# montib/rays1bench

Hardware: AMD Instinct MI355X
Metric: mrays/s on 'large' scene 1200x800x10spp (higher is better)
Workload: dtype f32

## Files before the change

include/rays1.h:

```cpp
#ifndef RAYS1_H
#define RAYS1_H

#include <stddef.h>
#include <stdint.h>

#ifdef __cplusplus
extern "C" {
#endif

#define R1_ABI_VERSION 4

enum
{
    R1_OK = 0,
    R1_EINVAL = -1,
    R1_ENODEVICE = -2,
    R1_EHIP = -3,
    R1_ENOMEM = -4,
    R1_ELIMIT = -5
};

enum
{
    R1_MAT_LAMBERTIAN = 0,
// ... 148 lines not shown


typedef struct r1_multi r1_multi;
int r1_multi_create(int32_t n_devices, const int32_t *devices, r1_multi **out);
void r1_multi_destroy(r1_multi *m);
int r1_multi_set_scene(r1_multi *m, const r1_scene *scene, const r1_camera *camera);
int r1_multi_set_camera(r1_multi *m, const r1_camera *camera);
int r1_multi_render(r1_multi *m, const r1_params *params, uint8_t *rgb_out, uint64_t *num_rays_out, double *device_seconds_out);
int r1_multi_render_async(r1_multi *m, const r1_params *params, void *host_frame);
int r1_multi_render_batch_async(r1_multi *m, const r1_params *params, int32_t n_frames, uint32_t seed_stride, void *host_frames);
int r1_multi_sync(r1_multi *m);
typedef struct r1_multi_layout_info
{
    size_t block_bytes;
    size_t record_bytes;
    size_t count_offset;
    size_t send_bytes;
    size_t gathered_bytes;
    size_t frame_record_bytes;
    size_t frame_count_offset;
    size_t host_bytes;
    size_t counts_pitch;
} r1_multi_layout_info;
int r1_multi_layout(const r1_params *params, int32_t n_devices, int32_t n_frames, r1_multi_layout_info *out);
int r1_multi_info(r1_multi *m, int32_t *n_devices, int32_t *rccl_version, r1_launch_info *first_device);


typedef struct r1_bvh_info
{
    int32_t nodes, leaves, depth, stack_entries, spheres, pairs;
    float centre[3];
    int32_t pad_local;
    int32_t root_leaf;
} r1_bvh_info;
int r1_bvh_describe(const r1_scene *scene, int32_t leaf_max, r1_bvh_info *info, float *nodes_out, size_t nodes_cap, uint32_t *ids_out,
                    size_t ids_cap);

typedef struct r1_grid_info
{
    float lo[3], hi[3];
    int32_t cells[3];
    float cell[3];
    float pad;
    float v_safe;
    float centre_lo[3], centre_hi[3];
    int32_t spheres;
    int32_t outliers;
    int32_t registrations;
    int32_t max_occupancy;
    float build_ms;
} r1_grid_info;
int r1_grid_describe(const r1_scene *scene, r1_grid_info *info, uint32_t *start_out, size_t start_cap, uint32_t *ids_out, size_t ids_cap,
                     uint32_t *outliers_out, size_t outliers_cap);

int r1_grid_visit(const r1_scene *scene, const float o[3], const float d[3], uint32_t *presented, size_t cap, size_t *n_presented,
                  int32_t *hit_index, float *hit_t, int32_t *fallback);

enum
{
    R1_SCENE_SMALL = 0,
    R1_SCENE_MEDIUM = 1,
    R1_SCENE_LARGE = 2,
    R1_SCENE_GRID = 3
};

typedef struct r1_host_scene r1_host_scene;
// ... 22 lines not shown
```

rays1bench_amd/binding.py:

```python
import ctypes as C
import os
import sys
import subprocess
import time

import numpy as np

_lib = None
HERE = os.path.dirname(os.path.abspath(__file__))
CSRC = os.path.join(HERE, "csrc")
LIBDIR = os.path.join(HERE, "lib")

R1_OK, R1_EINVAL, R1_ENODEVICE, R1_EHIP, R1_ENOMEM, R1_ELIMIT = 0, -1, -2, -3, -4, -5
SCENE_SMALL, SCENE_MEDIUM, SCENE_LARGE, SCENE_GRID = 0, 1, 2, 3
VARIANT_DEFAULT, VARIANT_REFERENCE, VARIANT_PREFILTER, VARIANT_STATS, VARIANT_BVH, VARIANT_BVH_STATS, VARIANT_WAVEFRONT = 0, 1, 2, 3, 4, 5, 6
VARIANT_GRID, VARIANT_GRID_STATS = 7, 8



def _stream_arg(stream_ptr):
    if stream_ptr:
        return C.c_void_p(stream_ptr)
    torch = sys.modules.get("torch")
    if torch is not None and torch.cuda.is_available() and torch.cuda.is_initialized():
# ... 13 lines not shown
    ] + [("mat_type", C.POINTER(C.c_uint8))] + [
        (n, C.POINTER(C.c_float)) for n in ("albedo_r", "albedo_g", "albedo_b", "mat_param")
    ]


class CCamera(C.Structure):
    _fields_ = [(n, C.c_float * 3) for n in ("origin", "lower_left", "horizontal", "vertical", "u", "v", "w")] + [
        ("lens_radius", C.c_float)
    ]


class Params(C.Structure):
    _fields_ = [
        ("width", C.c_int32), ("height", C.c_int32), ("spp", C.c_int32), ("max_bounces", C.c_int32),
        ("seed", C.c_uint32), ("tile_w", C.c_int32), ("tile_h", C.c_int32),
        ("shard", C.c_int32), ("num_shards", C.c_int32), ("variant", C.c_int32),
    ]


class MultiLayout(C.Structure):
    _fields_ = [(k, C.c_size_t) for k in ("block_bytes", "record_bytes", "count_offset", "send_bytes", "gathered_bytes", "frame_record_bytes",
                                          "frame_count_offset", "host_bytes", "counts_pitch")]


class LaunchInfo(C.Structure):
    _fields_ = [("compute_units", C.c_int32), ("blocks", C.c_int32), ("threads_per_block", C.c_int32),
                ("spheres_active", C.c_int32), ("spheres_padded", C.c_int32), ("groups", C.c_int32), ("samples", C.c_uint64),
                ("kernel", C.c_int32), ("bvh_nodes", C.c_int32), ("bvh_leaves", C.c_int32), ("bvh_depth", C.c_int32),
                ("tiles_in_kernel", C.c_int32)]


class BvhInfo(C.Structure):
    _fields_ = [("nodes", C.c_int32), ("leaves", C.c_int32), ("depth", C.c_int32), ("stack_entries", C.c_int32), ("spheres", C.c_int32),
                ("pairs", C.c_int32), ("centre", C.c_float * 3), ("pad_local", C.c_int32), ("root_leaf", C.c_int32)]


def make_params(width, height, spp, seed=10001, max_bounces=50, tile_w=32, tile_h=32, shard=0, num_shards=1, variant=0):
    return Params(width, height, spp, max_bounces, seed, tile_w, tile_h, shard, num_shards, variant)


_lib_path = os.path.join(LIBDIR, "librays1.so")


def lib_path():
    return _lib_path


def set_lib_path(path):
    global _lib_path
    if _lib is not None:
        raise R1Error(R1_EINVAL, "set_lib_path after the library was loaded")
    _lib_path = os.path.abspath(path)


def build(verbose=False):
    subprocess.check_call(["make", "-j4", "-C", CSRC] + ([] if verbose else ["-s"]))


class GridInfo(C.Structure):
    _fields_ = [("lo", C.c_float * 3), ("hi", C.c_float * 3), ("cells", C.c_int32 * 3), ("cell", C.c_float * 3), ("pad", C.c_float),
                ("v_safe", C.c_float), ("centre_lo", C.c_float * 3), ("centre_hi", C.c_float * 3), ("spheres", C.c_int32),
                ("outliers", C.c_int32), ("registrations", C.c_int32), ("max_occupancy", C.c_int32), ("build_ms", C.c_float)]


_u8p, _f32p, _u64p, _i32p, _dblp = (C.POINTER(t) for t in (C.c_uint8, C.c_float, C.c_uint64, C.c_int32, C.c_double))
_ctx = C.c_void_p
SYMBOLS = [
# ... 428 lines not shown


def shard_block_bytes(params):
    return int(lib().r1_shard_block_bytes(C.byref(params)))


def frame_record_bytes(params):
    return int(lib().r1_frame_record_bytes(C.byref(params)))


def shard_record_bytes(params):
    return int(lib().r1_shard_record_bytes(C.byref(params)))


def tile_count(params):
    a, b = C.c_int32(), C.c_int32()
    _check(lib().r1_tile_count(C.byref(params), C.byref(a), C.byref(b)))
    return int(a.value), int(b.value)


def multi_layout(params, n_devices, n_frames=1):
    out = MultiLayout()
    _check(lib().r1_multi_layout(C.byref(params), n_devices, n_frames, C.byref(out)))
    return {k: int(getattr(out, k)) for k, _ in MultiLayout._fields_}


def bvh_describe(cscene, leaf_max=0):
    info = BvhInfo()
    _check(lib().r1_bvh_describe(C.byref(cscene), leaf_max, C.byref(info), None, 0, None, 0))
    nodes = np.zeros((info.nodes, 16), np.float32)
    ids = np.zeros(max(2 * info.pairs, 2), np.uint32)
    _check(lib().r1_bvh_describe(C.byref(cscene), leaf_max, C.byref(info), nodes.ctypes.data_as(_f32p), nodes.size,
                                 ids.ctypes.data_as(C.POINTER(C.c_uint32)), ids.size))
    d = {k: int(getattr(info, k)) for k, _ in BvhInfo._fields_ if k != "centre"}
    d["centre"] = np.array(list(info.centre), np.float32)
    return d, nodes, ids[:2 * info.pairs]


def grid_describe(cscene):
    info = GridInfo()
    _check(lib().r1_grid_describe(C.byref(cscene), C.byref(info), None, 0, None, 0, None, 0))
    ncells = int(info.cells[0]) * int(info.cells[1]) * int(info.cells[2])
    start = np.zeros(ncells + 1, np.uint32)
    ids = np.zeros(max(info.registrations, 1), np.uint32)
    outl = np.zeros(max(info.outliers, 1), np.uint32)
    u32p = C.POINTER(C.c_uint32)
    _check(lib().r1_grid_describe(C.byref(cscene), C.byref(info), start.ctypes.data_as(u32p), start.size, ids.ctypes.data_as(u32p), ids.size,
                                  outl.ctypes.data_as(u32p), outl.size))
    d = {}
    for k, t in GridInfo._fields_:
        v = getattr(info, k)
        d[k] = np.array(list(v), np.float32 if k != "cells" else np.int64) if hasattr(v, "__len__") else v
    return d, start, ids[:info.registrations], outl[:info.outliers]


def grid_visit(cscene, o, d, cap=1 << 16):
    o = np.ascontiguousarray(o, np.float32)
    d = np.ascontiguousarray(d, np.float32)
    pres = np.zeros(cap, np.uint32)
    n, hi, ht, fb = C.c_size_t(), C.c_int32(), C.c_float(), C.c_int32()
    _check(lib().r1_grid_visit(C.byref(cscene), o.ctypes.data_as(_f32p), d.ctypes.data_as(_f32p), pres.ctypes.data_as(C.POINTER(C.c_uint32)), cap,
                               C.byref(n), C.byref(hi), C.byref(ht), C.byref(fb)))
    if n.value > cap:
        return grid_visit(cscene, o, d, int(n.value))
    return pres[:n.value], int(hi.value), float(ht.value), bool(fb.value)


# ... 47 lines not shown
```

rays1bench_amd/csrc/r1_bvh.cpp:

```cpp
#include <hip/hip_runtime.h>

#include "r1_device.h"
#include "../../include/rays1.h"

#include <algorithm>
#include <cmath>
#include <cstdint>
#include <cstdlib>
#include <cstring>
#include <vector>

struct R1Bvh
{
    std::vector<float> nodes;
    std::vector<float> prims;
    std::vector<uint32_t> ids;
    int max_depth = 0;
    uint32_t n_leaves = 0;
    float centre[3] = {0, 0, 0};
    int pad_local = 0;
    int root_leaf = 0;
};

namespace
{

struct Box
{
    double lo[3], hi[3];
    double clo[3], chi[3];
    double kmax;
    double rmax;
    double floor_pad;
    void clear()
    {
        for (int a = 0; a < 3; ++a)
            lo[a] = clo[a] = 1e300, hi[a] = chi[a] = -1e300;
        kmax = rmax = floor_pad = 0;
    }
    void merge(const Box &b)
    {
        for (int a = 0; a < 3; ++a)
        {
            lo[a] = std::min(lo[a], b.lo[a]), hi[a] = std::max(hi[a], b.hi[a]);
            clo[a] = std::min(clo[a], b.clo[a]), chi[a] = std::max(chi[a], b.chi[a]);
        }
        kmax = std::max(kmax, b.kmax), rmax = std::max(rmax, b.rmax), floor_pad = std::max(floor_pad, b.floor_pad);
    }
    double area() const
    {
        const double dx = hi[0] - lo[0], dy = hi[1] - lo[1], dz = hi[2] - lo[2];
        return dx * dy + dy * dz + dz * dx;
    }
};
// ... 164 lines not shown
            }
        }
        if (mid <= b || mid >= e)
        {
            mid = b + n / 2;
            const int a = axis;
            std::nth_element(order.begin() + b, order.begin() + mid, order.begin() + e, [&](uint32_t p, uint32_t q) {
                return sphere[p].clo[a] < sphere[q].clo[a] || (sphere[p].clo[a] == sphere[q].clo[a] && p < q);
            });
        }

        const uint32_t node = (uint32_t)(out->nodes.size() / 16);
        out->nodes.resize(out->nodes.size() + 16);
        out->max_depth = std::max(out->max_depth, depth + 1);
        const Box b0 = bound(b, mid), b1 = bound(mid, e);
        const uint32_t c0 = build(b, mid, depth + 1, b0);
        const uint32_t c1 = build(mid, e, depth + 1, b1);
        fill(node, b0, c0, b1, c1);
        return node;
    }

    void fill(uint32_t node, const Box &b0, uint32_t c0, const Box &b1, uint32_t c1)
    {
        float m0[3], e0[3], m1[3], e1[3];
        double w0, k0, w1, k1;
        encode(b0, m0, e0, w0, k0);
        encode(b1, m1, e1, w1, k1);
        float *p = &out->nodes[16 * (size_t)node];
        const double u = ldexp(1.0, -24), w2 = std::max(w0, w1), k = std::max(k0, k1);
        const double head = 1.0 + ldexp(1.0, -18);
        float A, K;
        if (!pad_local)
        {
            double g2 = 0;
            for (const float *m : {m0, m1})
            {
                double q = 0;
                for (int a = 0; a < 3; ++a)
                    q += ((double)m[a] - centre[a]) * ((double)m[a] - centre[a]);
                g2 = std::max(g2, q);
            }
            const double c1n = std::fabs(centre[0]) + std::fabs(centre[1]) + std::fabs(centre[2]);
            A = round_up((2.0 * w2 + u) * head), K = round_up((k + 2.0 * w2 * g2 + u * (1.0 + c1n)) * head);
        }
        else
        {
            double g2 = 0, mn2 = 0, M = 0, M0 = 0, M1 = 0;
            for (int a = 0; a < 3; ++a)
            {
                const double h = 0.5 * ((double)m0[a] - (double)m1[a]), mn = 0.5 * ((double)m0[a] + (double)m1[a]);
                g2 += h * h, mn2 += mn * mn;
                M0 = std::max(M0, std::fabs((double)m0[a])), M1 = std::max(M1, std::fabs((double)m1[a]));
            }
            M = M0 + M1;
            const double eps = std::min(1.0, std::max(1.0 / 64.0, std::sqrt(g2) / d_typ));
            const double a_loc = (0.25 * (1.0 + eps) * w2 + u / 8.0) * (1.0 + ldexp(1.0, -10));
            A = round_up(a_loc * head);
            K = round_up((k + (1.0 + 1.0 / eps) * w2 * g2 + u * (0.5 + std::sqrt(mn2)) + a_loc * 3075.0 * 288.0 * u * u * M * M) * head);
        }
        p[0] = m0[0], p[1] = m1[0], p[2] = m0[1], p[3] = m1[1];
        p[4] = m0[2], p[5] = m1[2], p[6] = e0[0], p[7] = e1[0];
        p[8] = e0[1], p[9] = e1[1], p[10] = e0[2], p[11] = e1[2];
        p[12] = A, p[13] = K;
        memcpy(&p[14], &c0, 4);
        memcpy(&p[15], &c1, 4);
    }
};

}

void r1_build_bvh(uint32_t na, const float *cx, const float *cy, const float *cz, const float *rsq, const double *rbound, int leaf_max,
                  R1Bvh &out)
{
    out.nodes.clear(), out.prims.clear(), out.ids.clear();
    out.max_depth = 0, out.n_leaves = 0;
    if (leaf_max < 1)
// ... 141 lines not shown
                }
            }
            if (order_new.size() == nn)
            {
                std::vector<uint32_t> new_of(nn);
                for (uint32_t i = 0; i < nn; ++i)
                    new_of[order_new[i]] = i;
                std::vector<float> moved(out.nodes.size());
                for (uint32_t i = 0; i < nn; ++i)
                {
                    memcpy(&moved[16 * (size_t)i], &out.nodes[16 * (size_t)order_new[i]], 64);
                    for (int c = 0; c < 2; ++c)
                    {
                        uint32_t r;
                        memcpy(&r, &moved[16 * (size_t)i + 14 + c], 4);
                        if (!(r & Builder::LEAF))
                        {
                            r = new_of[r];
                            memcpy(&moved[16 * (size_t)i + 14 + c], &r, 4);
                        }
                    }
                }
                out.nodes.swap(moved);
            }
        }
    }
    if (!B.pad_local)
    {
        const size_t nn = out.nodes.size() / 16;
        float a_max = 0.0f;
        for (size_t n = 0; n < nn; ++n)
            a_max = std::max(a_max, out.nodes[16 * n + 12]);
        for (size_t n = 0; n < nn; ++n)
        {
            float *q = &out.nodes[16 * n];
            const double K = q[13];
            for (int j = 6; j < 12; ++j)
                if (std::isfinite(q[j]))
                    q[j] = round_up((double)q[j] + K);
            q[12] = a_max, q[13] = 0.0f;
        }
    }
    out.root_leaf = 0;
    if (out.nodes.size() >= 16)
    {
        uint32_t c[2];
        memcpy(c, &out.nodes[14], 8);
        for (int k = 0; k < 2; ++k)
        {
            const uint32_t pairs = (c[k] >> 28) & 7u;
            if ((c[k] & Builder::LEAF) && !(c[1 - k] & Builder::LEAF) && pairs >= 1 && pairs <= 2)
                out.root_leaf = k + 1;
        }
    }
    if (out.prims.empty())
        out.prims.assign(8, 0.0f), out.ids.assign(2, 0xFFFFFFFFu);
}

extern "C" void r1_set_error(const char *fmt, ...);
int r1_active_spheres(const r1_scene *s, std::vector<uint32_t> &active_to_scene)
{
    active_to_scene.clear();
    for (uint32_t i = 0; i < s->count; ++i)
    {
        if (std::isnan(s->inv_radius[i]))
        {
            r1_set_error("scene: sphere %u has inv_radius NaN", i);
            return R1_EINVAL;
        }
        if (s->inv_radius[i] == 0)
            continue;
        if (!std::isfinite(s->center_x[i]) || !std::isfinite(s->center_y[i]) || !std::isfinite(s->center_z[i]) ||
            !std::isfinite(s->radius_sq[i]))
            continue;
        active_to_scene.push_back(i);
    }
    return R1_OK;
}

double r1_bound_radius(float radius_sq, float inv_radius)
{
    const double from_sq = radius_sq > 0 ? std::sqrt((double)radius_sq) : 0.0;
    const double from_inv = std::isfinite(inv_radius) && inv_radius != 0 ? 1.0 / std::fabs((double)inv_radius) : 0.0;
    return std::max(from_sq, from_inv);
}

extern "C" int r1_bvh_describe(const r1_scene *s, int32_t leaf_max, r1_bvh_info *info, float *nodes_out, size_t nodes_cap, uint32_t *ids_out,
                               size_t ids_cap)
{
    if (!s || !info || !s->center_x || !s->center_y || !s->center_z || !s->radius_sq || !s->inv_radius)
        return R1_EINVAL;
    std::vector<float> x, y, z, r;
    std::vector<double> rb;
    std::vector<uint32_t> scene_index;
    if (r1_active_spheres(s, scene_index) != R1_OK)
        return R1_EINVAL;
    for (uint32_t i : scene_index)
    {
        x.push_back(s->center_x[i]), y.push_back(s->center_y[i]), z.push_back(s->center_z[i]), r.push_back(s->radius_sq[i]);
        rb.push_back(r1_bound_radius(s->radius_sq[i], s->inv_radius[i]));
    }
    const uint32_t na = (uint32_t)x.size();
    if (na == 0)
        x.push_back(0), y.push_back(0), z.push_back(0), r.push_back(0), rb.push_back(0);
    R1Bvh b;
    r1_build_bvh(na, x.data(), y.data(), z.data(), r.data(), rb.data(),
                 leaf_max > 0 ? leaf_max : (na > R1_MAX_ACTIVE_10BIT ? 2 * R1_BVH_LEAF : R1_BVH_LEAF), b);
    info->nodes = (int32_t)(b.nodes.size() / 16);
    info->leaves = (int32_t)b.n_leaves;
    info->depth = b.max_depth;
    info->stack_entries = R1_BVH_STACK;
    info->spheres = (int32_t)na;
    for (int k = 0; k < 3; ++k)
        info->centre[k] = b.centre[k];
    info->pad_local = b.pad_local;
    info->root_leaf = b.root_leaf;
    if (nodes_out)
    {
        if (nodes_cap < b.nodes.size())
            return R1_ELIMIT;
        memcpy(nodes_out, b.nodes.data(), b.nodes.size() * 4);
    }
    info->pairs = (int32_t)(b.ids.size() / 2);
    if (ids_out)
    {
        if (ids_cap < b.ids.size())
            return R1_ELIMIT;
        for (size_t i = 0; i < b.ids.size(); ++i)
            ids_out[i] = b.ids[i] == 0xFFFFFFFFu || na == 0 ? 0xFFFFFFFFu : scene_index[b.ids[i]];
    }
    return R1_OK;
}
```

rays1bench_amd/csrc/r1_capi.cpp:

```cpp

#include <hip/hip_runtime.h>
#include <cmath>

#include <math.h>
#include <stdarg.h>
#include <stdio.h>
#include <stdlib.h>
#include <string.h>

#include <algorithm>
#include <new>
#include <utility>
#include <functional>
#include <vector>

#include "../../include/rays1.h"
#include "r1_device.h"
#include "r1_grid.h"

extern "C" hipError_t r1_launch_trace(const R1TraceArgs *args, int variant, int big, int mode, int path, int blocks, size_t grid_lds, hipStream_t stream);
extern "C" int r1_trace_mode(int variant, int big, int wanted);
extern "C" hipError_t r1_launch_resolve(const R1ResolveArgs *args, int max_rows, hipStream_t stream);
extern "C" hipError_t r1_launch_accum(const R1AccumArgs *args, hipStream_t stream);
extern "C" hipError_t r1_launch_wavefront(R1WaveArgs *w, int blocks, hipStream_t stream);
extern "C" hipError_t r1_launch_land_arm(uint32_t *tile_cnt, unsigned long long *frame_rays, uint32_t *frame_left, uint32_t n_frames, uint32_t n_local_tiles,
                                         int width, int height, int spp, int tile_w, int tile_h, int tiles_x, int shard, int num_shards, hipStream_t stream);
extern "C" hipError_t r1_launch_put6(void *dst, const uint32_t *words, hipStream_t stream);
extern "C" hipError_t r1_launch_put8(void *dst, const uint32_t *words, hipStream_t stream);
extern "C" hipError_t r1_launch_put_cameras(void *dst, const float *cameras20, int n, hipStream_t stream);
extern "C" hipError_t r1_launch_assemble(const void *blocks, void *rgb, int width, int height, int tile_w, int tile_h, int tiles_x, int num_shards,
                                         size_t shard_stride, int n_frames, size_t frame_in, size_t frame_out, size_t total_offset, long long total_out,
                                         int want_total, hipStream_t stream);
extern "C" size_t r1_frame_record_bytes(const r1_params *p);
extern "C" hipError_t r1_trace_occupancy(int variant, int big, int mode, size_t dyn_lds, int *blocks_per_cu);
extern "C" int r1_params_check(const r1_params *p);

struct R1Bvh
{
    std::vector<float> nodes;
    std::vector<float> prims;
    std::vector<uint32_t> ids;
    int max_depth = 0;
    uint32_t n_leaves = 0;
    float centre[3] = {0, 0, 0};
    int pad_local = 0;
    int root_leaf = 0;
};
void r1_build_bvh(uint32_t na, const float *cx, const float *cy, const float *cz, const float *rsq, const double *rbound, int leaf_max,
                  R1Bvh &out);
int r1_active_spheres(const r1_scene *s, std::vector<uint32_t> &active_to_scene);
double r1_bound_radius(float radius_sq, float inv_radius);


static thread_local char g_error[512] = "";

extern "C" void r1_set_error(const char *fmt, ...)
{
    va_list ap;
    va_start(ap, fmt);
    vsnprintf(g_error, sizeof(g_error), fmt, ap);
    va_end(ap);
}

extern "C" const char *r1_last_error(void) { return g_error; }
extern "C" int r1_abi_version(void) { return R1_ABI_VERSION; }

#define R1_HIP(call)                                                                                                   \
    do                                                                                                                 \
    {                                                                                                                  \
        hipError_t e_ = (call);                                                                                        \
        if (e_ != hipSuccess)                                                                                          \
        {                                                                                                              \
            r1_set_error("%s failed: %s (%s:%d)", #call, hipGetErrorString(e_), __FILE__, __LINE__);                   \
            return e_ == hipErrorOutOfMemory ? R1_ENOMEM : R1_EHIP;                                                    \
        }                                                                                                              \
    } while (0)


struct DevBuf
{
    void *p = nullptr;
    size_t cap = 0;
};

struct r1_context
{
    int device = 0;
    int cus = 0;
    hipStream_t stream = nullptr;
    hipEvent_t ev0 = nullptr, ev1 = nullptr, ev2 = nullptr;
    hipEvent_t last0 = nullptr, last1 = nullptr, last2 = nullptr;
    bool timing_valid = false;
    std::vector<hipEvent_t> ring;
    int ring_frames = 0, ring_used = 0;
    bool ring_on = false;

    DevBuf sweep, exact, exact_g, shade, mat, members;
    DevBuf bvh_nodes, bvh_prims, bvh_ids;
    DevBuf grid_tab, grid_out, grid_dev;
    DevBuf grid_tab32, grid_dev32;
    bool grid_valid = false;
    bool grid_small = false;
    R1GridArgs grid_args;
    DevBuf wf_paths, wf_hits, wf_queue, wf_counts;
    DevBuf wave_log;
    unsigned long long wave_log_ptr = 0;
    uint32_t wave_log_waves = 0;
    uint32_t n_bvh_nodes = 0, n_bvh_leaves = 0;
    int bvh_depth = 0;
    float bvh_centre[3] = {0, 0, 0};
    int bvh_pad_local = 0;
    int bvh_root_leaf = 0;
    uint32_t n_active = 0, n_sweep = 0, n_padded_scene = 0, n_groups = 0, n_multi = 0;
    std::vector<uint32_t> active_to_scene;
    R1DeviceCamera cam;
    bool have_scene = false;
    std::vector<float> src_f32[9];
    std::vector<uint8_t> src_mat;
    r1_camera src_cam;

    DevBuf counters, samples, image;
    R1BatchArgs batch_args_last = {0, 0, {0, 0, 0}, 0};
    hipStream_t batch_args_stream = nullptr;
    int batch_args_slot = -1;
    DevBuf path_cams;
    int path_cams_half = 0;
    bool land_prev = false;
    int land_parity = 0;
    uint32_t land_gen = 0;
    bool land_armed = false;
    r1_params land_key;
    int land_frames = 0;
    DevBuf batch_rays;
    int tile_frames = 0;
    bool counters_clean = false;
    r1_params tile_key;
    bool tile_key_valid = false;
    uint32_t n_local_tiles = 0, total_samples = 0, full = 0;

    unsigned long long *host_word = nullptr, *host_word_dev = nullptr;
    int default_variant = 4;
    int default_variant_tp = 4;
    int occupancy[160] = {0};
    bool pixel_mode = false;
    DevBuf gstack;
// ... 518 lines not shown
    R1_HIP(hipMemcpyAsync(c->mat.p, mat.data(), mat.size() * 4, hipMemcpyHostToDevice, c->stream));
    R1_HIP(hipMemcpyAsync(c->members.p, members.data(), members.size() * 4, hipMemcpyHostToDevice, c->stream));
    R1_HIP(hipMemcpyAsync(c->exact_g.p, exact_g.data(), exact_g.size() * 4, hipMemcpyHostToDevice, c->stream));
    R1_HIP(hipMemcpyAsync(c->bvh_nodes.p, bvh.nodes.data(), bvh.nodes.size() * 4, hipMemcpyHostToDevice, c->stream));
    R1_HIP(hipMemcpyAsync(c->bvh_prims.p, bvh.prims.data(), bvh.prims.size() * 4, hipMemcpyHostToDevice, c->stream));
    R1_HIP(hipMemcpyAsync(c->bvh_ids.p, bvh.ids.data(), bvh.ids.size() * 4, hipMemcpyHostToDevice, c->stream));
    R1_HIP(hipStreamSynchronize(c->stream));
    c->bvh_nodes_host = bvh.nodes;
    c->entry_valid = false;
    c->bvh_wide_f4 = 0;
    if (R1_BVH4 && bvh.nodes.size() >= 16 && bvh.nodes.size() / 16 <= R1_NODES_LDS_MAX && !bvh.pad_local)
    {
        std::vector<float> wide;
        c->bvh_wide_stack = build_wide(bvh.nodes, bvh.root_leaf, wide);
        if (c->bvh_wide_stack <= R1_BVH_STACK && wide.size() / 4 < 7u * 4096u)
        {
            if ((rc = ensure(c->bvh_wide, wide.size() * 4)))
                return rc;
            R1_HIP(hipMemcpy(c->bvh_wide.p, wide.data(), wide.size() * 4, hipMemcpyHostToDevice));
            c->bvh_wide_f4 = (uint32_t)(wide.size() / 4);
        }
        static const int print = (int)r1_knob("R1_BVH4_PRINT", 0);
        if (print)
            fprintf(stderr, "rays1: 4-wide table: %zu binary nodes -> %zu wide nodes, stack %d entries (binary: %d)\n", bvh.nodes.size() / 16, wide.size() / 28 - 1,
                    c->bvh_wide_stack, bvh.max_depth);
    }
    c->n_bvh_nodes = (uint32_t)(bvh.nodes.size() / 16);
    c->n_bvh_leaves = bvh.n_leaves;
    c->bvh_depth = bvh.max_depth;
    for (int k = 0; k < 3; ++k)
        c->bvh_centre[k] = bvh.centre[k];
    c->bvh_pad_local = bvh.pad_local;
    c->bvh_root_leaf = bvh.root_leaf;
    for (int &o : c->occupancy)
        o = 0;
    c->n_groups = ng;
    c->n_multi = n_multi;

    c->n_active = na;
    c->n_sweep = ns;
    c->n_padded_scene = s->count;
    c->cam = device_camera(*cam);
    for (int k = 0; k < 9; ++k)
        c->src_f32[k].assign(src[k], src[k] + s->count);
    c->src_mat.assign(s->mat_type, s->mat_type + s->count);
    c->src_cam = *cam;
    c->have_scene = true;
    c->default_variant = c->default_variant_tp = 4;
    return R1_OK;
}

extern "C" int r1_set_camera(r1_context *c, const r1_camera *cam)
{
    if (!c || !cam)
    {
        r1_set_error("r1_set_camera: %s is NULL", !c ? "ctx" : "camera");
        return R1_EINVAL;
    }
    if (!c->have_scene)
    {
        r1_set_error("r1_set_camera: no scene set (call r1_set_scene first)");
        return R1_EINVAL;
    }
    c->pass_valid = false;
    c->cam = device_camera(*cam);
    c->src_cam = *cam;
// ... 354 lines not shown
        const size_t cols = ((size_t)p->tile_w * p->tile_h + 255) / 256;
        if ((rc = ensure(c->batch_rays, (size_t)n_frames * (c->n_local_tiles ? c->n_local_tiles : 1) * cols * 8)))
            return rc;
    }
    const bool land = variant == 4 && R1_LAND_MODE(mode) && c->total_samples > 0;
    if (!pixel_mode)
    {
        const size_t want = (size_t)(c->total_samples ? c->total_samples : 1) * 16;
        const bool fresh = !c->samples.p || c->samples.cap < want;
        if ((rc = ensure(c->samples, want)))
            return rc;
        if (fresh)
            R1_HIP(hipMemsetAsync(c->samples.p, 0, c->samples.cap, st));
    }

    R1TraceArgs a;
    memset(&a, 0, sizeof(a));
    a.scene.sweep = (const float4 *)c->sweep.p;
    a.scene.exact = (const float4 *)c->exact.p;
    a.scene.shade = (const float4 *)c->shade.p;
    a.scene.mat = (const float4 *)c->mat.p;
    a.scene.members = (const uint32_t *)c->members.p;
    a.scene.exact_g = (const float4 *)c->exact_g.p;
    a.scene.n_active = c->n_active;
    a.scene.n_sweep = c->n_sweep;
    a.scene.n_multi = c->n_multi;
    a.scene.bvh_nodes = (const float4 *)c->bvh_nodes.p;
    a.scene.bvh_prims = (const float4 *)c->bvh_prims.p;
    a.scene.bvh_ids = (const uint32_t *)c->bvh_ids.p;
    for (int k = 0; k < 3; ++k)
        a.scene.bvh_centre[k] = c->bvh_centre[k];
    a.scene.bvh_pad_local = (uint32_t)c->bvh_pad_local;
    a.scene.bvh_root_leaf = (uint32_t)c->bvh_root_leaf;
    a.cam = c->cam;
    a.width = p->width, a.height = p->height, a.spp = p->spp, a.max_bounces = p->max_bounces;
    a.seed = p->seed;
    a.inv_w = 1.0f / p->width;
    a.inv_h = 1.0f / p->height;
    a.tile_w = p->tile_w, a.tile_h = p->tile_h;
    a.tiles_x = (p->width + p->tile_w - 1) / p->tile_w;
    a.shard = p->shard, a.num_shards = p->num_shards;
    a.n_local_tiles = c->n_local_tiles;
    a.batch = nullptr;
    const bool path = batch && batch->cameras && n_frames > 1;
    if (batch && batch->cameras && n_frames == 1)
        a.cam = device_camera(batch->cameras[0]);
    if (path)
    {
        const size_t half = ((size_t)n_frames * R1_PATH_CAM_F4 * 16 + 255) & ~(size_t)255;
        if ((rc = ensure(c->path_cams, 2 * half)))
            return rc;
        c->path_cams_half ^= 1;
        char *const table = (char *)c->path_cams.p + (c->path_cams_half ? c->path_cams.cap / 2 : 0);
        std::vector<float> rows((size_t)n_frames * R1_PATH_CAM_F4 * 4, 0.0f);
        for (int f = 0; f < n_frames; ++f)
        {
            const R1DeviceCamera d = device_camera(batch->cameras[f]);
            static_assert(sizeof(R1DeviceCamera) == 19 * 4 && R1_PATH_CAM_F4 * 4 >= 19, "a table row holds an R1DeviceCamera");
            memcpy(&rows[(size_t)f * R1_PATH_CAM_F4 * 4], &d, sizeof(d));
        }
        R1_HIP(r1_launch_put_cameras(table, rows.data(), n_frames, st));
        R1PathArgs pa;
        memset(&pa, 0, sizeof(pa));
        pa.batch.n_frames = (uint32_t)n_frames, pa.batch.seed_stride = batch->seed_stride;
        pa.batch.div_tiles = make_div(c->n_local_tiles ? c->n_local_tiles : 1u), pa.batch.n_local_tiles = c->n_local_tiles;
        pa.cameras = (const float *)table;
// ... 934 lines not shown
```

rays1bench_amd/csrc/r1_device.h:

```cpp
#ifndef R1_DEVICE_H
#define R1_DEVICE_H

#include <stdint.h>

#include "r1_grid_dda.h"

#define R1_BLOCK 256
#define R1_BIT_WORDS 8
#define R1_CAND_CAP 16
#define R1_PAIR_CAP 1024
#define R1_PAIR_CAP_SMALL 512
#define R1_STACK_WORDS 17
#ifndef R1_STACK_LDS_WORDS
#define R1_STACK_LDS_WORDS 10
#endif
#ifndef R1_STACK_LDS_WORDS_TP
#define R1_STACK_LDS_WORDS_TP 10
#endif
#define R1_RESOLVE_ROWS_TP 256
#define R1_NODES_LDS_MAX 256
#define R1_CHUNK 256
#define R1_CHUNK_BIG 1024
#define R1_CHUNK_MIN 32
#define R1_GROUP_MAX 4
// ... 94 lines not shown
    uint8_t *out;
    unsigned long long *rays_dst;
    unsigned long long out_stride;
    unsigned long long rays_offset;
    unsigned long long *frame_rays;
    uint32_t *frame_left;
    uint32_t *clear_heads;
    uint32_t clear_count;
    uint32_t n_frames;
    uint32_t rays_in_out, block_layout;
    float inv_spp;
    uint32_t *owed_spill;
    uint32_t spill_stride;
    uint32_t *error;
};

struct R1DeviceScene
{
    const float4 *sweep;
    const float4 *exact;
    const float4 *shade;
    const float4 *exact_g;
    const uint32_t *members;
    const float4 *mat;
    uint32_t n_multi;
    uint32_t n_active;
    uint32_t n_sweep;
    const float4 *bvh_nodes;
    const float4 *bvh_prims;
    const uint32_t *bvh_ids;
    float bvh_centre[3];
    uint32_t bvh_pad_local;
    uint32_t bvh_root_leaf;
};

struct R1GridArgs
{
    R1GridGeom geom;
    const uint32_t *outliers;
    uint32_t n_out;
    uint32_t n_start;
    const uint32_t *tab;
    uint32_t lds_bytes;
};

struct R1DeviceCamera
{
    float origin[3], lower_left[3], horizontal[3], vertical[3], u[3], v[3];
    float lens_radius;
};

struct R1TraceArgs
{
    R1DeviceScene scene;
    R1DeviceCamera cam;
    int32_t width, height, spp, max_bounces;
    uint32_t seed;
    float inv_w, inv_h;
    int32_t tile_w, tile_h, tiles_x;
    int32_t shard, num_shards;
    uint32_t n_local_tiles;
    const struct R1BatchArgs *batch;
    uint32_t full;
    R1FastDiv div_full, div_spp, div_tw, div_tx;
    uint32_t total_samples;
    uint32_t chunk_min, chunk_max;
// ... 72 lines not shown
```

rays1bench_amd/csrc/r1_trace.hpp:

```cpp
#ifndef R1_TRACE_HPP
#define R1_TRACE_HPP


#include <hip/hip_runtime.h>
#include <float.h>
#include <stdint.h>

#include "r1_device.h"
#include "r1_grid_dda.h"
#include "../../include/rays1_seed.h"

#pragma clang fp contract(off)

namespace
{

struct V3
{
    float x, y, z;
};

typedef float f4 __attribute__((ext_vector_type(4)));
typedef const f4 __attribute__((address_space(4))) *cf4_ptr;
typedef float v2f __attribute__((ext_vector_type(2)));
// ... 566 lines not shown

__device__ __forceinline__ void trav_put(uint32_t *trav, const int at, const uint32_t ref) { trav[at] = ref; }
__device__ __forceinline__ uint32_t trav_get(const uint32_t *trav, const int at) { return trav[at]; }
__device__ __forceinline__ void trav_put(uint16_t *trav, const int at, const uint32_t ref) { trav[at] = (uint16_t)ref; }
__device__ __forceinline__ uint32_t trav_get(const uint16_t *trav, const int at) { return trav[at]; }
__device__ __forceinline__ uint32_t r1_ref16(const uint32_t ref) { return ((ref >> 16) & 0xF000u) | (ref & 0x0FFFu); }

struct Trav
{
    uint32_t cur;
    int sp;
    float best;
    uint32_t best_id;
};

__device__ __forceinline__ void trav_start(Trav &t)
{
    t.cur = 0u, t.sp = 0, t.best = FLT_MAX, t.best_id = 0xFFFFFFFFu;
}

#ifndef R1_CARRY_DIV
#define R1_CARRY_DIV 6u
#endif
template <bool STATS, bool CARRY, bool LN, typename TS, bool ENTRY = false>
__device__ __forceinline__ void bvh_advance(const R1DeviceScene &S, const V3 o, const V3 d, Trav &tv, TS *trav, const int tid,
                                            const uint32_t n_alive, unsigned long long *wstat, const float4 *lnodes , const uint32_t top = 0u ,
                                            const uint32_t *entry_tab = nullptr, const uint32_t entry_idx = 0xFFFFFFFFu, const uint16_t *entry_lds = nullptr )
{
    const float4 *__restrict__ nodes = S.bvh_nodes;
    const float4 *__restrict__ prims = S.bvh_prims;
    const uint32_t *__restrict__ ids = S.bvh_ids;
    const V3 inv = mk(__builtin_amdgcn_rcpf(d.x), __builtin_amdgcn_rcpf(d.y), __builtin_amdgcn_rcpf(d.z));
    const V3 ainv = mk(fabsf(inv.x), fabsf(inv.y), fabsf(inv.z));
    const V3 oi = mk(o.x * inv.x, o.y * inv.y, o.z * inv.z);
    const float rx = o.x - S.bvh_centre[0], ry = o.y - S.bvh_centre[1], rz = o.z - S.bvh_centre[2];
    const float r2 = __fmaf_rn(rz, rz, __fmaf_rn(ry, ry, rx * rx));
    V3 pa_ray = mk(0.0f, 0.0f, 0.0f);
    if (LN)
    {
        const float pad_ray = lnodes[3].x * r2;
        pa_ray = mk(pad_ray * ainv.x, pad_ray * ainv.y, pad_ray * ainv.z);
    }
    float best = tv.best;
    uint32_t best_id = tv.best_id;
    uint32_t cur = tv.cur;
    int sp = tv.sp;
    constexpr uint32_t LEAF_BIT = LN ? 0x8000u : 0x80000000u, INDEX_MASK = LN ? 0x0FFFu : 0x0FFFFFFFu;
    constexpr int COUNT_SHIFT = LN ? 12 : 28;
    auto visit_node = [&]() {
        if (STATS)
        {
            wstat[9] += 1;
            if ((tid & 63) == __ffsll((long long)__ballot(1)) - 1)
                wstat[2] += 1;
        }
#if R1_BVH4
        if (LN)
        {
            uint32_t at = 7u * cur;
            const uint4 rf = *(const uint4 *)(lnodes + at + 6u);
            float t0, t1, t2, t3;
            float4 q0 = lnodes[at + 0u], q1 = lnodes[at + 1u], q2 = lnodes[at + 2u];
            const bool g0 = bvh_box(q0.x, q0.z, q1.x, q1.z, q2.x, q2.z, pa_ray, oi, inv, ainv, best, t0);
            const bool g1 = bvh_box(q0.y, q0.w, q1.y, q1.w, q2.y, q2.w, pa_ray, oi, inv, ainv, best, t1);
            uint32_t k0 = g0 ? ((__float_as_uint(fmaxf(t0, 0.0f)) & 0xFFFF0000u) | rf.x) : 0xFFFFFFFFu;
            uint32_t k1 = g1 ? ((__float_as_uint(fmaxf(t1, 0.0f)) & 0xFFFF0000u) | rf.y) : 0xFFFFFFFFu;
            asm volatile("" : "+v"(at), "+v"(k0), "+v"(k1));
// ... 35 lines not shown
            q3 = nodes[4 * (size_t)cur + 3];
        float tn0, tn1;
        V3 pa = pa_ray;
        if (!LN)
        {
            float dist2 = r2;
            if (S.bvh_pad_local)
            {
                const float sx = __fmaf_rn(-2.0f, o.x, q0.x + q0.y), sy = __fmaf_rn(-2.0f, o.y, q0.z + q0.w), sz = __fmaf_rn(-2.0f, o.z, q1.x + q1.y);
                dist2 = __fmaf_rn(sz, sz, __fmaf_rn(sy, sy, sx * sx));
            }
            const float pad = __fmaf_rn(q3.x, dist2, q3.y);
            pa = mk(pad * ainv.x, pad * ainv.y, pad * ainv.z);
        }
        const bool h0 = bvh_box(q0.x, q0.z, q1.x, q1.z, q2.x, q2.z, pa, oi, inv, ainv, best, tn0);
        const bool h1 = bvh_box(q0.y, q0.w, q1.y, q1.w, q2.y, q2.w, pa, oi, inv, ainv, best, tn1);
        const uint32_t c0 = __float_as_uint(q3.z), c1 = __float_as_uint(q3.w);
        if (h0 && h1)
        {
            const bool swap = tn1 < tn0;
            trav_put(trav, sp * R1_BLOCK + tid, swap ? c0 : c1);
            ++sp;
            cur = swap ? c1 : c0;
        }
        else if (h0)
            cur = c0;
        else if (h1)
            cur = c1;
        else if (sp > 0)
            cur = trav_get(trav, --sp * R1_BLOCK + tid);
        else
            cur = R1_BVH_DONE;
    };
    const uint32_t root_leaf = LN ? __float_as_uint(lnodes[3].y) : S.bvh_root_leaf;
    if (root_leaf != 0u && cur == 0u)
    {
        const int k = root_leaf == 1u ? 1 : 0;
        const float *nf = (const float *)lnodes;
        const uint32_t leaf = __float_as_uint(nf[14 + (1 - k)]);
        uint32_t other = __float_as_uint(nf[14 + k]);
        const uint32_t lp = (leaf >> COUNT_SHIFT) & 7u;
        if (STATS)
        {
            wstat[5] += (unsigned long long)lp, wstat[16] += 1ull, wstat[17] += 1ull;
            if ((tid & 63) == __ffsll((long long)__ballot(1)) - 1)
                wstat[3] += 1;
        }
        leaf_quad(prims, ids, leaf & INDEX_MASK, lp, o, d, best, best_id);
        V3 pa = pa_ray;
        if (!LN)
        {
            float dist2 = r2;
            if (S.bvh_pad_local)
            {
                const float sx = __fmaf_rn(-2.0f, o.x, nf[0] + nf[1]), sy = __fmaf_rn(-2.0f, o.y, nf[2] + nf[3]), sz = __fmaf_rn(-2.0f, o.z, nf[4] + nf[5]);
                dist2 = __fmaf_rn(sz, sz, __fmaf_rn(sy, sy, sx * sx));
            }
            const float pad = __fmaf_rn(nf[12], dist2, nf[13]);
            pa = mk(pad * ainv.x, pad * ainv.y, pad * ainv.z);
        }
        float tn;
        const bool h = bvh_box(nf[0 + k], nf[2 + k], nf[4 + k], nf[6 + k], nf[8 + k], nf[10 + k], pa, oi, inv, ainv, best, tn);
        if (ENTRY && entry_idx != 0xFFFFFFFFu && h)
        {
            if (LN && entry_lds != nullptr)
            {
                other = entry_lds[entry_idx];
                other = other == 0xFFFFu ? R1_BVH_DONE : other;
            }
            else
                other = ((const r1_gu32 *)entry_tab)[entry_idx];
        }
        cur = h ? other : R1_BVH_DONE;
    }
#if R1_BVH4
    if (LN && cur == 0u)
        cur = 1u;
#endif
    for (;;)
    {
        const unsigned long long walking = __ballot(cur != R1_BVH_DONE);
        if (walking == 0ull)
            break;
        if (CARRY && R1_CARRY_DIV * (uint32_t)__popcll(walking) <= n_alive)
            break;
        while (cur < LEAF_BIT)
            visit_node();
        if (cur != R1_BVH_DONE)
        {
            const uint32_t first = cur & INDEX_MASK, cnt = (cur >> COUNT_SHIFT) & 7u;
            for (uint32_t j = 0; j < cnt; j += 2u)
            {
                const uint32_t take = cnt - j < 2u ? 1u : 2u;
                if (STATS)
                {
                    wstat[5] += (unsigned long long)take;
                    wstat[16] += 1ull;
                    if ((tid & 63) == __ffsll((long long)__ballot(1)) - 1)
                        wstat[3] += 1;
                }
                leaf_quad(prims, ids, first + j, take, o, d, best, best_id);
            }
            cur = sp > 0 ? trav_get(trav, --sp * R1_BLOCK + tid) : R1_BVH_DONE;
        }
    }
    tv.cur = cur, tv.sp = sp, tv.best = best, tv.best_id = best_id;
}

template <bool STATS>
__device__ __forceinline__ void sweep_bvh(const R1DeviceScene &S, const bool alive, const V3 o, const V3 d, float &t_max, int &hit_index,
                                          uint32_t *trav, const int tid, unsigned long long *wstat)
{
    Trav tv;
    trav_start(tv);
    if (!alive)
        tv.cur = R1_BVH_DONE;
    bvh_advance<STATS, false, false, uint32_t>(S, o, d, tv, trav, tid, 64u, wstat, nullptr);
    if (tv.best_id != 0xFFFFFFFFu)
    {
        t_max = tv.best;
        hit_index = (int)tv.best_id;
    }
}

template <bool STATS, bool SMALL>
__device__ __forceinline__ bool grid_trace(const R1TraceArgs &GA, R1GridCArgs *G, const bool alive, const V3 o, const V3 d,
                                           float &best, uint32_t &best_id, const uint16_t *ltab, const int tid, unsigned long long *wstat)
{
    R1GridCArgs &geom_args = *G;
    auto &geom = geom_args.geom;
    best = FLT_MAX, best_id = 0xFFFFFFFFu;
    if (!alive)
        return false;
    for (uint32_t k = 0; k < G->n_out; ++k)
    {
        const uint32_t id = ((const __attribute__((address_space(4))) uint32_t *)G->outliers)[k];
// ... 630 lines not shown
    __shared__ f4 s_tile[BIG && VARIANT == 2 ? 2 * R1_TILE_F4 : 1];

    const int tid = (int)threadIdx.x;
    const int lane = tid & 63;

    constexpr bool LN = VARIANT == 4 && !BIG;
    typedef typename IdxType<!LN>::type TS;
    const size_t trav_words = VARIANT == 4 ? (size_t)A.bvh_depth * R1_BLOCK * sizeof(TS) / 4 : 0;
    const size_t gtrav_words = VARIANT == 7 ? (size_t)A.bvh_depth * R1_BLOCK : 0;
    const uint16_t *ltab = (const uint16_t *)(s_trav + gtrav_words);
    if (VARIANT == 7 && !BIG)
    {
        float4 *dst = (float4 *)(s_trav + gtrav_words);
        const R1GridCArgs *ga = (const R1GridCArgs *)(uintptr_t)A.grid;
        const float4 *src = (const float4 *)(const r1_gu32 *)ga->tab;
        const uint32_t n16 = ga->lds_bytes / 16u;
        for (uint32_t i = (uint32_t)tid; i < n16; i += R1_BLOCK)
            dst[i] = src[i];
        __syncthreads();
    }
    const float4 *lnodes = (const float4 *)(s_trav + trav_words);
    const uint32_t top = LN ? 0u : A.bvh_lds_f4 >> 2;
    if (VARIANT == 4 && A.bvh_lds_f4)
    {
        float4 *dst = (float4 *)(s_trav + trav_words);
        for (uint32_t i = (uint32_t)tid; i < A.bvh_lds_f4; i += R1_BLOCK)
        {
            float4 q = (R1_BVH4 && LN) ? A.bvh_wide[i] : A.scene.bvh_nodes[i];
            if (LN && !R1_BVH4 && (i & 3u) == 3u)
                q.z = __uint_as_float(r1_ref16(__float_as_uint(q.z))), q.w = __uint_as_float(r1_ref16(__float_as_uint(q.w)));
            dst[i] = q;
        }
        if (LN && tid == 3)
            ((float *)dst)[13] = __uint_as_float(A.scene.bvh_root_leaf);
        if (LN && !BATCH && R1_ENTRY_MODE(MODE) && A.entry_lds)
            for (uint32_t i = (uint32_t)tid; i < A.entry_lds; i += R1_BLOCK)
                ((uint16_t *)(dst + A.bvh_lds_f4))[i] = (uint16_t)A.bvh_entry[i];
        __syncthreads();
    }

    Path p;
    p.o = mk(0, 0, 0), p.d = mk(0, 0, 0);
    p.s_scalar = p.s0 = p.s1 = p.s2 = 1;
    p.k = 0, p.depth = 0, p.sp = 0;
    bool alive = false;
    Pixel px;
    px.acc = mk(0, 0, 0), px.xy = 0, px.off = 0, px.s = (uint32_t)A.spp;
    Trav tv;
    trav_start(tv);
    tv.cur = R1_BVH_DONE;
    unsigned long long lane_rays = 0;
#ifndef R1_SPARE
#define R1_SPARE 1
#endif
#ifndef R1_SPARE_MIN
#define R1_SPARE_MIN 40u
#endif
    constexpr bool SPARE = R1_SPARE && !BIG && (VARIANT == 4 || VARIANT == 2 || VARIANT == 7) && (MODE == 0 || MODE == 3 || MODE == 5);
    Path spare = p;
    bool has_spare = false;

    uint32_t q_next = 0, q_end = 0;
    const uint32_t q_total = A.total_samples;
    uint32_t q_remaining = q_total;
    const uint32_t n_waves2 = 2u * n_tb * (R1_BLOCK / 64);
    uint32_t *const q_head = LAND ? A.queue + 32u * xcd : A.queue;
    constexpr uint32_t LAND_GROUP = LAT ? 8u : 1u;
// ... 372 lines not shown
```

Baseline: 37400.

## Add flat-axis BVH traversal that tests the y slab once per ray

```diff
diff --git a/include/rays1.h b/include/rays1.h
--- a/include/rays1.h
+++ b/include/rays1.h
@@ -204,6 +204,8 @@
     float centre[3];
     int32_t pad_local;
     int32_t root_leaf;
+    int32_t flat_axis;
+    float flat_m, flat_e;
 } r1_bvh_info;
 int r1_bvh_describe(const r1_scene *scene, int32_t leaf_max, r1_bvh_info *info, float *nodes_out, size_t nodes_cap, uint32_t *ids_out,
                     size_t ids_cap);
diff --git a/rays1bench_amd/binding.py b/rays1bench_amd/binding.py
--- a/rays1bench_amd/binding.py
+++ b/rays1bench_amd/binding.py
@@ -69,7 +69,8 @@
 
 class BvhInfo(C.Structure):
     _fields_ = [("nodes", C.c_int32), ("leaves", C.c_int32), ("depth", C.c_int32), ("stack_entries", C.c_int32), ("spheres", C.c_int32),
-                ("pairs", C.c_int32), ("centre", C.c_float * 3), ("pad_local", C.c_int32), ("root_leaf", C.c_int32)]
+                ("pairs", C.c_int32), ("centre", C.c_float * 3), ("pad_local", C.c_int32), ("root_leaf", C.c_int32),
+                ("flat_axis", C.c_int32), ("flat_m", C.c_float), ("flat_e", C.c_float)]
 
 
 def make_params(width, height, spp, seed=10001, max_bounces=50, tile_w=32, tile_h=32, shard=0, num_shards=1, variant=0):
@@ -564,7 +565,8 @@
     ids = np.zeros(max(2 * info.pairs, 2), np.uint32)
     _check(lib().r1_bvh_describe(C.byref(cscene), leaf_max, C.byref(info), nodes.ctypes.data_as(_f32p), nodes.size,
                                  ids.ctypes.data_as(C.POINTER(C.c_uint32)), ids.size))
-    d = {k: int(getattr(info, k)) for k, _ in BvhInfo._fields_ if k != "centre"}
+    d = {k: int(getattr(info, k)) for k, _ in BvhInfo._fields_ if k not in ("centre", "flat_m", "flat_e")}
+    d["flat_m"], d["flat_e"] = np.float32(info.flat_m), np.float32(info.flat_e)
     d["centre"] = np.array(list(info.centre), np.float32)
     return d, nodes, ids[:2 * info.pairs]
 
diff --git a/rays1bench_amd/csrc/r1_bvh.cpp b/rays1bench_amd/csrc/r1_bvh.cpp
--- a/rays1bench_amd/csrc/r1_bvh.cpp
+++ b/rays1bench_amd/csrc/r1_bvh.cpp
@@ -20,6 +20,8 @@
     float centre[3] = {0, 0, 0};
     int pad_local = 0;
     int root_leaf = 0;
+    int flat_axis = -1;
+    float flat_m = 0, flat_e = 0;
 };
 
 namespace
@@ -250,16 +252,28 @@
         float A, K;
         if (!pad_local)
         {
-            double g2 = 0;
+            static const int child_k = (int)r1_knob("R1_BVH_CHILD_K", 1);
+            const double c1n = std::fabs(centre[0]) + std::fabs(centre[1]) + std::fabs(centre[2]);
+            double g2c[2], kc[2] = {k0, k1}, wc[2] = {w0, w1};
+            int j = 0;
             for (const float *m : {m0, m1})
             {
                 double q = 0;
                 for (int a = 0; a < 3; ++a)
                     q += ((double)m[a] - centre[a]) * ((double)m[a] - centre[a]);
-                g2 = std::max(g2, q);
-            }
-            const double c1n = std::fabs(centre[0]) + std::fabs(centre[1]) + std::fabs(centre[2]);
-            A = round_up((2.0 * w2 + u) * head), K = round_up((k + 2.0 * w2 * g2 + u * (1.0 + c1n)) * head);
+                g2c[j++] = q;
+            }
+            if (!child_k)
+                g2c[0] = g2c[1] = std::max(g2c[0], g2c[1]), kc[0] = kc[1] = k, wc[0] = wc[1] = w2;
+            A = round_up((2.0 * w2 + u) * head), K = 0.0f;
+            j = 0;
+            for (float *e : {e0, e1})
+            {
+                const float Kc = round_up((kc[j] + 2.0 * wc[j] * g2c[j] + u * (1.0 + c1n)) * head);
+                for (int a = 0; a < 3; ++a)
+                    e[a] = round_up((double)e[a] + (double)Kc);
+                ++j;
+            }
         }
         else
         {
@@ -467,14 +481,7 @@
         for (size_t n = 0; n < nn; ++n)
             a_max = std::max(a_max, out.nodes[16 * n + 12]);
         for (size_t n = 0; n < nn; ++n)
-        {
-            float *q = &out.nodes[16 * n];
-            const double K = q[13];
-            for (int j = 6; j < 12; ++j)
-                if (std::isfinite(q[j]))
-                    q[j] = round_up((double)q[j] + K);
-            q[12] = a_max, q[13] = 0.0f;
-        }
+            out.nodes[16 * n + 12] = a_max;
     }
     out.root_leaf = 0;
     if (out.nodes.size() >= 16)
@@ -486,6 +493,36 @@
             const uint32_t pairs = (c[k] >> 28) & 7u;
             if ((c[k] & Builder::LEAF) && !(c[1 - k] & Builder::LEAF) && pairs >= 1 && pairs <= 2)
                 out.root_leaf = k + 1;
+        }
+    }
+    out.flat_axis = -1, out.flat_m = out.flat_e = 0.0f;
+    {
+        static const double ratio_env = r1_knob_f("R1_BVH_FLAT_RATIO", 1.25);
+        const size_t nn = out.nodes.size() / 16;
+        if (ratio_env > 0 && !B.pad_local && nn >= 2 && nn <= R1_NODES_LDS_MAX && na <= R1_MAX_ACTIVE_10BIT)
+        {
+            double best_ratio = 1e300;
+            for (int a : {1, 0, 2})
+            {
+                double L = 1e300, H = -1e300, narrow = 1e300;
+                for (size_t n = out.root_leaf ? 1 : 0; n < nn; ++n)
+                    for (int c = 0; c < 2; ++c)
+                    {
+                        const double m = out.nodes[16 * n + 2 * a + c], e = out.nodes[16 * n + 6 + 2 * a + c];
+                        if (!(e >= 0))
+                            continue;
+                        L = std::min(L, m - e), H = std::max(H, m + e), narrow = std::min(narrow, 2.0 * e);
+                    }
+                if (!(H >= L) || !(narrow > 0) || !std::isfinite(H - L))
+                    continue;
+                const double ratio = (H - L) / narrow;
+                if (ratio <= ratio_env && ratio < best_ratio)
+                {
+                    best_ratio = ratio;
+                    const float mu = (float)(0.5 * (L + H));
+                    out.flat_axis = a, out.flat_m = mu, out.flat_e = round_up(std::max(H - (double)mu, (double)mu - L));
+                }
+            }
         }
     }
     if (out.prims.empty())
@@ -550,6 +587,7 @@
         info->centre[k] = b.centre[k];
     info->pad_local = b.pad_local;
     info->root_leaf = b.root_leaf;
+    info->flat_axis = b.flat_axis, info->flat_m = b.flat_m, info->flat_e = b.flat_e;
     if (nodes_out)
     {
         if (nodes_cap < b.nodes.size())
diff --git a/rays1bench_amd/csrc/r1_capi.cpp b/rays1bench_amd/csrc/r1_capi.cpp
--- a/rays1bench_amd/csrc/r1_capi.cpp
+++ b/rays1bench_amd/csrc/r1_capi.cpp
@@ -45,6 +45,8 @@
     float centre[3] = {0, 0, 0};
     int pad_local = 0;
     int root_leaf = 0;
+    int flat_axis = -1;
+    float flat_m = 0, flat_e = 0;
 };
 void r1_build_bvh(uint32_t na, const float *cx, const float *cy, const float *cz, const float *rsq, const double *rbound, int leaf_max,
                   R1Bvh &out);
@@ -111,6 +113,7 @@
     float bvh_centre[3] = {0, 0, 0};
     int bvh_pad_local = 0;
     int bvh_root_leaf = 0;
+    float bvh_flat_m = 0.0f, bvh_flat_e = -1.0f;
     uint32_t n_active = 0, n_sweep = 0, n_padded_scene = 0, n_groups = 0, n_multi = 0;
     std::vector<uint32_t> active_to_scene;
     R1DeviceCamera cam;
@@ -695,6 +698,7 @@
         c->bvh_centre[k] = bvh.centre[k];
     c->bvh_pad_local = bvh.pad_local;
     c->bvh_root_leaf = bvh.root_leaf;
+    c->bvh_flat_m = bvh.flat_axis == 1 ? bvh.flat_m : 0.0f, c->bvh_flat_e = bvh.flat_axis == 1 ? bvh.flat_e : -1.0f;
     for (int &o : c->occupancy)
         o = 0;
     c->n_groups = ng;
@@ -1115,6 +1119,7 @@
         a.scene.bvh_centre[k] = c->bvh_centre[k];
     a.scene.bvh_pad_local = (uint32_t)c->bvh_pad_local;
     a.scene.bvh_root_leaf = (uint32_t)c->bvh_root_leaf;
+    a.scene.bvh_flat_m = c->bvh_flat_m, a.scene.bvh_flat_e = c->bvh_flat_e;
     a.cam = c->cam;
     a.width = p->width, a.height = p->height, a.spp = p->spp, a.max_bounces = p->max_bounces;
     a.seed = p->seed;
diff --git a/rays1bench_amd/csrc/r1_device.h b/rays1bench_amd/csrc/r1_device.h
--- a/rays1bench_amd/csrc/r1_device.h
+++ b/rays1bench_amd/csrc/r1_device.h
@@ -150,6 +150,7 @@
     float bvh_centre[3];
     uint32_t bvh_pad_local;
     uint32_t bvh_root_leaf;
+    float bvh_flat_m, bvh_flat_e;
 };
 
 struct R1GridArgs
diff --git a/rays1bench_amd/csrc/r1_trace.hpp b/rays1bench_amd/csrc/r1_trace.hpp
--- a/rays1bench_amd/csrc/r1_trace.hpp
+++ b/rays1bench_amd/csrc/r1_trace.hpp
@@ -622,7 +622,7 @@
     const uint32_t *__restrict__ ids = S.bvh_ids;
     const V3 inv = mk(__builtin_amdgcn_rcpf(d.x), __builtin_amdgcn_rcpf(d.y), __builtin_amdgcn_rcpf(d.z));
     const V3 ainv = mk(fabsf(inv.x), fabsf(inv.y), fabsf(inv.z));
-    const V3 oi = mk(o.x * inv.x, o.y * inv.y, o.z * inv.z);
+    V3 oi = mk(o.x * inv.x, o.y * inv.y, o.z * inv.z);
     const float rx = o.x - S.bvh_centre[0], ry = o.y - S.bvh_centre[1], rz = o.z - S.bvh_centre[2];
     const float r2 = __fmaf_rn(rz, rz, __fmaf_rn(ry, ry, rx * rx));
     V3 pa_ray = mk(0.0f, 0.0f, 0.0f);
@@ -724,7 +724,40 @@
         else
             cur = R1_BVH_DONE;
     };
-    const uint32_t root_leaf = LN ? __float_as_uint(lnodes[3].y) : S.bvh_root_leaf;
+    constexpr bool FLAT_OK = LN && !ENTRY && !R1_BVH4;
+    auto visit_flat = [&]() {
+        if (STATS)
+        {
+            wstat[9] += 1;
+            if ((tid & 63) == __ffsll((long long)__ballot(1)) - 1)
+                wstat[2] += 1;
+        }
+        const float4 q0 = lnodes[4 * cur + 0], q1 = lnodes[4 * cur + 1], q2 = lnodes[4 * cur + 2], q3 = lnodes[4 * cur + 3];
+        const float ax0 = __fmaf_rn(q0.x, inv.x, -oi.x), az0 = __fmaf_rn(q1.x, inv.z, -oi.z);
+        const float bx0 = __fmaf_rn(q1.z, ainv.x, pa_ray.x), bz0 = __fmaf_rn(q2.z, ainv.z, pa_ray.z);
+        const float ax1 = __fmaf_rn(q0.y, inv.x, -oi.x), az1 = __fmaf_rn(q1.y, inv.z, -oi.z);
+        const float bx1 = __fmaf_rn(q1.w, ainv.x, pa_ray.x), bz1 = __fmaf_rn(q2.w, ainv.z, pa_ray.z);
+        const float tn0 = fmaxf(fmaxf(ax0 - bx0, az0 - bz0), oi.y), tf0 = fminf(fminf(ax0 + bx0, az0 + bz0), pa_ray.y);
+        const float tn1 = fmaxf(fmaxf(ax1 - bx1, az1 - bz1), oi.y), tf1 = fminf(fminf(ax1 + bx1, az1 + bz1), pa_ray.y);
+        const bool h0 = tn0 <= tf0, h1 = tn1 <= tf1;
+        const uint32_t c0 = __float_as_uint(q3.z), c1 = __float_as_uint(q3.w);
+        if (h0 && h1)
+        {
+            const bool swap = tn1 < tn0;
+            trav_put(trav, sp * R1_BLOCK + tid, swap ? c0 : c1);
+            ++sp;
+            cur = swap ? c1 : c0;
+        }
+        else if (h0)
+            cur = c0;
+        else if (h1)
+            cur = c1;
+        else if (sp > 0)
+            cur = trav_get(trav, --sp * R1_BLOCK + tid);
+        else
+            cur = R1_BVH_DONE;
+    };
+    const uint32_t root_leaf = LN ? __float_as_uint(lnodes[3].y) & 3u : S.bvh_root_leaf;
     if (root_leaf != 0u && cur == 0u)
     {
         const int k = root_leaf == 1u ? 1 : 0;
@@ -769,6 +802,14 @@
     if (LN && cur == 0u)
         cur = 1u;
 #endif
+    if (FLAT_OK && (__builtin_amdgcn_readfirstlane((int)__float_as_uint(lnodes[3].y)) & 4) != 0)
+    {
+        const float a_u = __fmaf_rn(lnodes[7].x, inv.y, -oi.y), b_u = __fmaf_rn(lnodes[7].y, ainv.y, pa_ray.y);
+        const float tyf = a_u + b_u;
+        oi.y = fmaxf(a_u - b_u, 0.0f);
+        pa_ray.y = tyf < best ? tyf : best;
+        cur = oi.y <= pa_ray.y ? cur : R1_BVH_DONE;
+    }
     for (;;)
     {
         const unsigned long long walking = __ballot(cur != R1_BVH_DONE);
@@ -776,8 +817,12 @@
             break;
         if (CARRY && R1_CARRY_DIV * (uint32_t)__popcll(walking) <= n_alive)
             break;
-        while (cur < LEAF_BIT)
-            visit_node();
+        if (FLAT_OK && (__builtin_amdgcn_readfirstlane((int)__float_as_uint(lnodes[3].y)) & 4) != 0)
+            while (cur < LEAF_BIT)
+                visit_flat();
+        else
+            while (cur < LEAF_BIT)
+                visit_node();
         if (cur != R1_BVH_DONE)
         {
             const uint32_t first = cur & INDEX_MASK, cnt = (cur >> COUNT_SHIFT) & 7u;
@@ -794,6 +839,8 @@
                 leaf_quad(prims, ids, first + j, take, o, d, best, best_id);
             }
             cur = sp > 0 ? trav_get(trav, --sp * R1_BLOCK + tid) : R1_BVH_DONE;
+            if (FLAT_OK && (__builtin_amdgcn_readfirstlane((int)__float_as_uint(lnodes[3].y)) & 4) != 0)
+                pa_ray.y = best < pa_ray.y ? best : pa_ray.y;
         }
     }
     tv.cur = cur, tv.sp = sp, tv.best = best, tv.best_id = best_id;
@@ -1490,7 +1537,9 @@
             dst[i] = q;
         }
         if (LN && tid == 3)
-            ((float *)dst)[13] = __uint_as_float(A.scene.bvh_root_leaf);
+            ((float *)dst)[13] = __uint_as_float(A.scene.bvh_root_leaf | ((!R1_BVH4 && A.scene.bvh_flat_e >= 0.0f) ? 4u : 0u));
+        if (LN && !R1_BVH4 && tid == 7 && A.scene.bvh_flat_e >= 0.0f)
+            ((float *)dst)[28] = A.scene.bvh_flat_m, ((float *)dst)[29] = A.scene.bvh_flat_e;
         if (LN && !BATCH && R1_ENTRY_MODE(MODE) && A.entry_lds)
             for (uint32_t i = (uint32_t)tid; i < A.entry_lds; i += R1_BLOCK)
                 ((uint16_t *)(dst + A.bvh_lds_f4))[i] = (uint16_t)A.bvh_entry[i];
```

Result: faster. 38560, median of 6 (+3.1%).
